# spencerkent/vision-transform-codes

Hardware: AMD Instinct MI355X
Metric: patches/sec through 200-iter FISTA + dict update, 1024-atom dict (higher is better)
Workload: dtype f16x3

## Files before the change

### vision-transform-codes_amd/csrc/fc_fused.hip

```cpp
#include "fc_fused.h"
#include "fused_common.h"

#include <stdlib.h>
#include <mutex>
#include <vector>

namespace vtc {

struct FusedParams {
  const float* images;
  const float* init;
  float* codes;
  const uint4* packA[2];
  const uint4* packT[2];
  const float* betas;
  int64_t b;
  int s;
  int num_iters;
  int fista;
  float eta, cutoff;
  const float* eta_dev;
  float lam;
  const float* dscale;
  unsigned long long* stamps;
// ... 355 lines not shown
      const float cn = Y[p][e] + Gp[e];
      Y[p][e] = cn;
      cn4[k] = cn;
      if (k == 3) {
        if (p < CREG) {
#pragma unroll
          for (int q = 0; q < 4; ++q) Cr[p < CREG ? p : 0][4 * g + q] = cn4[q];
        } else {
          *reinterpret_cast<float4*>(Cst + cst_ln + (p - CREG) * 16384 +
                                     g * 1024) =
              make_float4(cn4[0], cn4[1], cn4[2], cn4[3]);
        }
      }
      return;
    }
    if (k == 0) {
      if (p < CREG) {
        cold4 = make_float4(Cr[p < CREG ? p : 0][4 * g + 0],
                            Cr[p < CREG ? p : 0][4 * g + 1],
                            Cr[p < CREG ? p : 0][4 * g + 2],
                            Cr[p < CREG ? p : 0][4 * g + 3]);
      } else {
        cold4 = *reinterpret_cast<const float4*>(
            Cst + cst_ln + (p - CREG) * 16384 + g * 1024);
      }
    }
    const float co = (k == 0) ? cold4.x : (k == 1) ? cold4.y
                   : (k == 2) ? cold4.z : cold4.w;
    const float c = sub_rn(Y[p][e], mul_rn(eta, Gp[e]));
    const float cn = shrink_fast<MODE>(c, cutoff_l);
    Y[p][e] = fista ? add_rn(cn, mul_rn(beta, sub_rn(cn, co))) : cn;
    cn4[k] = cn;
    if (k == 3) {
      if (p < CREG) {
#pragma unroll
        for (int q = 0; q < 4; ++q) Cr[p < CREG ? p : 0][4 * g + q] = cn4[q];
      } else {
        *reinterpret_cast<float4*>(Cst + cst_ln + (p - CREG) * 16384 +
                                   g * 1024) =
            make_float4(cn4[0], cn4[1], cn4[2], cn4[3]);
      }
      const float v4[4] = {Y[p][4 * g], Y[p][4 * g + 1], Y[p][4 * g + 2],
                           Y[p][4 * g + 3]};
      uint2 hi, lo;
      split_packed<F16, 4, NP == 2>(v4, hi, lo);
      char* dst = Yx + (p & 1) * NP * kYxPart + yx_wr + 16 * g;
      *reinterpret_cast<uint2*>(dst) = hi;
      if (NP == 2) *reinterpret_cast<uint2*>(dst + kYxPart) = lo;
    }
  };

  auto step1 = [&](int p, int sg, bool overlap, float beta) {
    f32x16& G = Gb[p & 1];
#pragma unroll
    for (int e = 0; e < 16; ++e) G[e] = 0.f;
    uint4 rb_next[NP];
#pragma unroll
    for (int part = 0; part < NP; ++part)
      rb_next[part] =
          *reinterpret_cast<const uint4*>(Rx + part * kRxPart + rx_rd);
#pragma unroll
    for (int i = 0; i < 16; ++i) {
      uint4 rb[NP];
#pragma unroll
      for (int part = 0; part < NP; ++part) {
        rb[part] = rb_next[part];
        if (i + 1 < 16)
          rb_next[part] = *reinterpret_cast<const uint4*>(
              Rx + part * kRxPart + rx_rd + 32 * (i + 1));
      }
      G = mfma16<F16>(ring[0][i % RING], rb[0], G);
      if constexpr (NP == 2) {
        G = mfma16<F16>(ring[0][i % RING], rb[1], G);
        G = mfma16<F16>(ring[1][i % RING], rb[0], G);
      }
      if (overlap) {
        epilogue_elem(p - 1, i, Gb[(p - 1) & 1], beta);
        __builtin_amdgcn_sched_barrier(0);
      }
      VTC_REFILL(sg, i)
      __builtin_amdgcn_sched_barrier(0);
    }
  };

  for (int it = 0; it < P.num_iters; ++it) {
    const float beta = fista ? P.betas[it] : 0.f;
    step1(0, 0, false, beta);
    VTC_STAMP(0)
#pragma unroll
    for (int p = 0; p < NPH; ++p) {
      if (p + 1 < NPH) {
        step1(p + 1, 2 * p + 1, true, beta);
        VTC_STAMP(0)
      }
      __syncthreads();
      VTC_STAMP(2)
      if (p + 2 == NPH) {
        step3(p, p & 1, true, 2 * p + 2, [&](int i) {
          epilogue_elem(NPH - 1, i, Gb[(NPH - 1) & 1], beta);
          __builtin_amdgcn_sched_barrier(0);
        });
      } else {
        step3(p, p & 1, true, (p + 1 < NPH) ? 2 * p + 2 : 2 * NPH - 1, nothing);
      }
      VTC_STAMP(3)
    }
    exchange_r();
    VTC_STAMP(4)
  }
  if (STAMP && lane == 0) {
#pragma unroll
    for (int k = 0; k < 5; ++k) atomicAdd(P.stamps + k, acc_t[k]);
    atomicAdd(P.stamps + 7, 1ull);
  }
#undef VTC_STAMP

#pragma unroll
  for (int p = 0; p < NPH; ++p) {
#pragma unroll
    for (int g = 0; g < 4; ++g) {
      float4 v;
      if (p < CREG) {
        v = make_float4(Cr[p < CREG ? p : 0][4 * g + 0],
                        Cr[p < CREG ? p : 0][4 * g + 1],
                        Cr[p < CREG ? p : 0][4 * g + 2],
                        Cr[p < CREG ? p : 0][4 * g + 3]);
      } else {
        v = *reinterpret_cast<const float4*>(Cst + cst_ln +
                                             (p - CREG) * 16384 + g * 1024);
      }
      if (F16) {
        v.x *= inv_sigma_y;
        v.y *= inv_sigma_y;
        v.z *= inv_sigma_y;
        v.w *= inv_sigma_y;
      }
      if (live)
        *reinterpret_cast<float4*>(P.codes + patch * s + kPhaseAtoms * p +
                                   32 * w + 8 * g + 4 * h) = v;
    }
  }
#undef VTC_LOAD_A
#undef VTC_LOAD_T
#undef VTC_LOAD_SEG
#undef VTC_REFILL
#undef VTC_SEG_IS_T
#undef VTC_SEG_PHASE
}

template <int NPH, int NP, int MODE, bool F16 = false, bool STAMP = false,
          int SCHED = 0>
__global__ __launch_bounds__(256, 1) void fused_fista_kernel16(FusedParams P) {
  static_assert(!F16 || NP == 2, "the f16 split exists as three products only");
  static_assert(SCHED >= 0 && SCHED < 4, "two schedule bits");
  constexpr bool SPREAD = (SCHED & 1) != 0 && NPH > 2;
  constexpr bool EARLY_R = (SCHED & 2) != 0;
  using L = FusedLds<NPH, NP>;
  constexpr int CREG = L::CREG;
  constexpr int CR = CREG > 0 ? CREG : 1;
  constexpr int RING = (NP == 1) ? 16 : 8;
  constexpr int NPROD = (NP == 2) ? 3 : 1;
  extern __shared__ __attribute__((aligned(16))) char smem[];
  char* Cst = smem;
  char* Yx = smem + L::cst_bytes;
  char* Rx = Yx + L::yx_bytes;
  float* Stat = reinterpret_cast<float*>(Rx + L::rx_bytes);

  const int tid = threadIdx.x;
  const int lane = tid & 63;
  const int w = __builtin_amdgcn_readfirstlane(tid >> 6);
  const int c = lane & 15, q = lane >> 4;
  int64_t patch[2];
  bool live[2];
#pragma unroll
  for (int n = 0; n < 2; ++n) {
    patch[n] = (int64_t)blockIdx.x * kFP + 16 * n + c;
    live[n] = patch[n] < P.b;
  }
  const int s = P.s;

  const unsigned pack_bytes_total = (unsigned)s * kFN * 2u;
  const unsigned a_wave_off = (unsigned)w * (16u * 64u * 16u);
  const unsigned t_wave_off = (unsigned)(4 * w) * (4u * 64u * 16u);
  __amdgpu_buffer_rsrc_t rsA[NP], rsT[NP];
#pragma unroll
  for (int part = 0; part < NP; ++part) {
    rsA[part] = __builtin_amdgcn_make_buffer_rsrc(
        (void*)((const char*)P.packA[part] + a_wave_off), 0,
        (int)(pack_bytes_total - a_wave_off), 0x00020000);
    rsT[part] = __builtin_amdgcn_make_buffer_rsrc(
        (void*)((const char*)P.packT[part] + t_wave_off), 0,
        (int)(pack_bytes_total - t_wave_off), 0x00020000);
  }
  const unsigned frag_voff = (unsigned)lane * 16u;
#define VTC_LOAD_A(part, p, i) \
  buffer_load16(rsA[part], frag_voff, (unsigned)(((4 * (p)) * 16 + (i)) * 1024))
#define VTC_LOAD_T(part, p, nb, ks) \
  buffer_load16(rsT[part], frag_voff,  \
                (unsigned)((((p) * 16 + (nb)) * 4 + (ks)) * 1024))

  const int swap = ((c >> 2) ^ (c >> 3)) & 1;
  const int rd_chunk = 32 * (q >> 1) + 16 * ((q & 1) ^ swap);
  const int wr_chunk = 16 * ((q >> 1) ^ swap) + 8 * (q & 1);
  const int yx_rd = c * kYxRow + rd_chunk;
  const int yx_wr = c * kYxRow + 64 * w + wr_chunk;
  const int rx_rd = c * kRxRow + rd_chunk;
  const int rx_wr = c * kRxRow + 128 * w + wr_chunk;
  const int cst_ln = w * 4096 + lane * 16;
  constexpr int kYxHalf = 16 * kYxRow, kRxHalf = 16 * kRxRow;

  f32x16 Y[NPH];
  f32x16 Cr[CR];
  f32x4 Xr[4][2];
  f32x4 Racc[4][2];
  uint4 ring[NP][RING];

#pragma unroll
  for (int nb = 0; nb < 4; ++nb) {
#pragma unroll
    for (int n = 0; n < 2; ++n) {
      float4 v = make_float4(0.f, 0.f, 0.f, 0.f);
      if (live[n])
        v = *reinterpret_cast<const float4*>(P.images + patch[n] * kFN + 64 * w +
                                             16 * nb + 4 * q);
      Xr[nb][n][0] = v.x;
      Xr[nb][n][1] = v.y;
      Xr[nb][n][2] = v.z;
      Xr[nb][n][3] = v.w;
    }
  }
  const bool warm = (P.init != nullptr);
#pragma unroll
  for (int p = 0; p < NPH; ++p) {
#pragma unroll
    for (int g = 0; g < 4; ++g) {
      float4 v = make_float4(0.f, 0.f, 0.f, 0.f);
      if (warm && live[g & 1])
        v = *reinterpret_cast<const float4*>(P.init + patch[g & 1] * s +
                                             kPhaseAtoms * p + 32 * w +
                                             16 * (g >> 1) + 4 * q);
      Y[p][4 * g + 0] = v.x;
      Y[p][4 * g + 1] = v.y;
      Y[p][4 * g + 2] = v.z;
      Y[p][4 * g + 3] = v.w;
    }
  }
  float sigma_y[2] = {1.f, 1.f}, inv_sigma_y[2] = {1.f, 1.f};
  float sigma_d = 1.f, inv_sigma_d = 1.f;
  if (F16) {
    float sx[2] = {0.f, 0.f}, sy[2] = {0.f, 0.f};
#pragma unroll
    for (int nb = 0; nb < 4; ++nb)
#pragma unroll
      for (int n = 0; n < 2; ++n)
#pragma unroll
        for (int k = 0; k < 4; ++k) sx[n] += Xr[nb][n][k] * Xr[nb][n][k];
    if (warm) {
#pragma unroll
      for (int p = 0; p < NPH; ++p)
#pragma unroll
        for (int e = 0; e < 16; ++e) sy[(e >> 2) & 1] += Y[p][e] * Y[p][e];
    }
    float* red = reinterpret_cast<float*>(Rx);
#pragma unroll
    for (int n = 0; n < 2; ++n) {
      sx[n] += __shfl_xor(sx[n], 16, 64);
      sx[n] += __shfl_xor(sx[n], 32, 64);
      sy[n] += __shfl_xor(sy[n], 16, 64);
      sy[n] += __shfl_xor(sy[n], 32, 64);
      if (q == 0) {
        red[w * 64 + 16 * n + c] = sx[n];
        red[w * 64 + 32 + 16 * n + c] = sy[n];
      }
    }
    __syncthreads();
    float m2[2];
#pragma unroll
    for (int n = 0; n < 2; ++n) {
      float tx = 0.f, ty = 0.f;
#pragma unroll
      for (int v = 0; v < 4; ++v) {
        tx += red[v * 64 + 16 * n + c];
        ty += red[v * 64 + 32 + 16 * n + c];
      }
      m2[n] = fmaxf(tx, ty);
    }
    __syncthreads();
    sigma_d = P.dscale[0];
    inv_sigma_d = P.dscale[1];
#pragma unroll
    for (int n = 0; n < 2; ++n) {
      int e2 = 0;
      if (m2[n] > 0.f && m2[n] < __builtin_inff()) e2 = ilogbf(m2[n]) >> 1;
      e2 = e2 < -60 ? -60 : (e2 > 60 ? 60 : e2);
      sigma_y[n] = ldexpf(1.f, 8 - e2);
      inv_sigma_y[n] = ldexpf(1.f, e2 - 8);
      const float sx_scale = sigma_d * sigma_y[n];
#pragma unroll
      for (int nb = 0; nb < 4; ++nb)
#pragma unroll
        for (int k = 0; k < 4; ++k) Xr[nb][n][k] *= sx_scale;
    }
#pragma unroll
    for (int p = 0; p < NPH; ++p)
#pragma unroll
      for (int e = 0; e < 16; ++e) Y[p][e] *= sigma_y[(e >> 2) & 1];
  }
  float eta = P.eta, cutoff = P.cutoff;
  if (P.eta_dev) {
    eta = *P.eta_dev;
    cutoff = mul_rn(P.lam, eta);
  }
  float cutoff_l[2] = {cutoff, cutoff};
  if (F16) {
    eta = eta * (0.5f * inv_sigma_d);
    cutoff_l[0] = cutoff * sigma_y[0];
    cutoff_l[1] = cutoff * sigma_y[1];
  }
  const float r_scale = F16 ? 2.f * inv_sigma_d : 1.f;
  int xr_calls = 0;
#pragma unroll
  for (int p = 0; p < NPH; ++p) {
#pragma unroll
    for (int g = 0; g < 4; ++g) {
      if (p < CREG) {
#pragma unroll
        for (int k = 0; k < 4; ++k)
          Cr[p < CREG ? p : 0][4 * g + k] = Y[p][4 * g + k];
      } else {
        *reinterpret_cast<float4*>(Cst + cst_ln + (p - CREG) * 16384 +
                                   g * 1024) =
            make_float4(Y[p][4 * g + 0], Y[p][4 * g + 1], Y[p][4 * g + 2],
                        Y[p][4 * g + 3]);
      }
    }
  }
#pragma unroll
  for (int nb = 0; nb < 4; ++nb)
#pragma unroll
    for (int n = 0; n < 2; ++n)
#pragma unroll
      for (int k = 0; k < 4; ++k) Racc[nb][n][k] = 0.f;

  auto publish_group = [&](const f32x16& y, int g, int buf) {
    const float v4[4] = {y[4 * g], y[4 * g + 1], y[4 * g + 2], y[4 * g + 3]};
    uint2 hi, lo;
    split_packed<F16, 4, NP == 2>(v4, hi, lo);
    char* dst = Yx + buf * NP * kYxPart + yx_wr + 32 * (g >> 1) +
                kYxHalf * (g & 1);
    *reinterpret_cast<uint2*>(dst) = hi;
    if (NP == 2) *reinterpret_cast<uint2*>(dst + kYxPart) = lo;
  };

#define VTC_SEG_IS_T(sg) (((sg) >= 2 && ((sg) % 2) == 0) || (sg) == 2 * NPH - 1)
#define VTC_SEG_PHASE(sg)                                        \
  ((sg) == 0 ? 0                                                 \
             : (sg) == 2 * NPH - 1 ? NPH - 1                     \
                                   : ((sg) % 2 ? ((sg) + 1) / 2 : (sg) / 2 - 1))
#define VTC_SEG_BLOCK_MAJOR(sg) (EARLY_R && (sg) == 2 * NPH - 1)
#define VTC_T_NB(sg, i) \
  (VTC_SEG_BLOCK_MAJOR(sg) ? 2 * ((i) >> 3) + ((i) & 1) : (i) & 3)
#define VTC_T_KS(sg, i) (VTC_SEG_BLOCK_MAJOR(sg) ? ((i) >> 1) & 3 : (i) >> 2)
#define VTC_LOAD_SEG(part, sg, i)                                          \
  (VTC_SEG_IS_T(sg) ? VTC_LOAD_T(part, VTC_SEG_PHASE(sg), VTC_T_NB(sg, i), \
                                 VTC_T_KS(sg, i))                          \
                    : VTC_LOAD_A(part, VTC_SEG_PHASE(sg), (i)))
#define VTC_REFILL(sg, i)                                                   \
  {                                                                         \
    const int j_ = (i) + RING;                                              \
    const int sg_ = (j_ < 16) ? (sg) : (((sg) + 1) % (2 * NPH));            \
    const int i_ = (j_ < 16) ? j_ : j_ - 16;                                \
    _Pragma("unroll") for (int part = 0; part < NP; ++part)                 \
        ring[part][(i) % RING] = VTC_LOAD_SEG(part, sg_, i_);               \
  }
#define VTC_MFMA_PAIR(acc0, acc1, a, b)                                     \
  _Pragma("unroll") for (int prod = 0; prod < NPROD; ++prod) {              \
    acc0 = mfma_k32<F16>(a[prod == 2], b[0][prod == 1], acc0);              \
    acc1 = mfma_k32<F16>(a[prod == 2], b[1][prod == 1], acc1);              \
  }

  auto step3 = [&](int p, int buf, bool pipe, int sg, auto&& between) {
    uint4 yb[2][NP], yb_next[2][NP];
#pragma unroll
    for (int n = 0; n < 2; ++n)
#pragma unroll
      for (int part = 0; part < NP; ++part)
        yb_next[n][part] = *reinterpret_cast<const uint4*>(
            Yx + (buf * NP + part) * kYxPart + yx_rd + kYxHalf * n);
#pragma unroll
    for (int i = 0; i < 16; ++i) {
      const int ks = i >> 2, nb = i & 3;
      if (nb == 0) {
#pragma unroll
        for (int n = 0; n < 2; ++n)
#pragma unroll
          for (int part = 0; part < NP; ++part) yb[n][part] = yb_next[n][part];
      }
      if (nb < 2 && ks + 1 < 4) {
#pragma unroll
        for (int part = 0; part < NP; ++part)
          yb_next[nb][part] = *reinterpret_cast<const uint4*>(
              Yx + (buf * NP + part) * kYxPart + yx_rd + kYxHalf * nb +
              64 * (ks + 1));
      }
      uint4 a[NP];
#pragma unroll
      for (int part = 0; part < NP; ++part)
        a[part] = pipe ? ring[part][i % RING] : VTC_LOAD_T(part, p, nb, ks);
      VTC_MFMA_PAIR(Racc[nb][0], Racc[nb][1], a, yb)
      between(i);
      if (pipe) VTC_REFILL(sg, i)
      __builtin_amdgcn_sched_barrier(0);
    }
  };
  auto nothing = [](int) {};

  auto exchange_r = [&]() {
    float v[4][2][4];
#pragma unroll
    for (int nb = 0; nb < 4; ++nb)
#pragma unroll
      for (int n = 0; n < 2; ++n)
#pragma unroll
        for (int k = 0; k < 4; ++k) {
          v[nb][n][k] = sub_rn(Racc[nb][n][k], Xr[nb][n][k]);
          if (F16) v[nb][n][k] *= r_scale;
        }
    if (F16) {
      float f[2] = {1.f, 1.f};
#pragma unroll
      for (int n = 0; n < 2; ++n) {
        float m = 0.f;
#pragma unroll
        for (int nb = 0; nb < 4; ++nb)
#pragma unroll
          for (int k = 0; k < 4; ++k) m = fmaxf(m, fabsf(v[nb][n][k]));
        m = fmaxf(m, __shfl_xor(m, 16, 64));
        m = fmaxf(m, __shfl_xor(m, 32, 64));
        const int row = 16 * n + c;
        if (xr_calls > 0) {
          const float* prev = Stat + ((xr_calls - 1) & 1) * 128;
          const float Mx = fmaxf(fmaxf(prev[row], prev[32 + row]),
                                 fmaxf(prev[64 + row], prev[96 + row]));
          if (Mx > 2048.f && Mx < __builtin_inff())
            f[n] = ldexpf(1.f, 9 - ilogbf(Mx));
        }
        if (q == 0) Stat[(xr_calls & 1) * 128 + w * 32 + row] = m * f[n];
      }
      ++xr_calls;
      if (__any(f[0] != 1.f || f[1] != 1.f)) {
#pragma unroll
        for (int p = 0; p < NPH; ++p)
#pragma unroll
          for (int e = 0; e < 16; ++e) Y[p][e] *= f[(e >> 2) & 1];
#pragma unroll
        for (int p = 0; p < CR; ++p)
#pragma unroll
          for (int e = 0; e < 16; ++e) Cr[p][e] *= f[(e >> 2) & 1];
#pragma unroll
        for (int pl = 0; pl < L::CL; ++pl)
#pragma unroll
          for (int g = 0; g < 4; ++g) {
            float4* c4 = reinterpret_cast<float4*>(Cst + cst_ln + pl * 16384 +
                                                   g * 1024);
            float4 cc = *c4;
            const float fg = f[g & 1];
            cc.x *= fg; cc.y *= fg; cc.z *= fg; cc.w *= fg;
            *c4 = cc;
          }
#pragma unroll
        for (int n = 0; n < 2; ++n) {
#pragma unroll
          for (int nb = 0; nb < 4; ++nb)
#pragma unroll
            for (int k = 0; k < 4; ++k) {
              Xr[nb][n][k] *= f[n];
              v[nb][n][k] *= f[n];
            }
          cutoff_l[n] *= f[n];
          inv_sigma_y[n] *= 1.f / f[n];
        }
      }
    }
#pragma unroll
    for (int nb = 0; nb < 4; ++nb) {
#pragma unroll
      for (int n = 0; n < 2; ++n) {
        const float v4[4] = {v[nb][n][0], v[nb][n][1], v[nb][n][2], v[nb][n][3]};
        uint2 hi, lo;
        split_packed<F16, 4, NP == 2>(v4, hi, lo);
        char* dst = Rx + rx_wr + 32 * nb + kRxHalf * n;
        *reinterpret_cast<uint2*>(dst) = hi;
        if (NP == 2) *reinterpret_cast<uint2*>(dst + kRxPart) = lo;
      }
    }
#pragma unroll
    for (int nb = 0; nb < 4; ++nb)
#pragma unroll
      for (int n = 0; n < 2; ++n)
#pragma unroll
        for (int k = 0; k < 4; ++k) Racc[nb][n][k] = 0.f;
    __syncthreads();
  };

  float xf[2] = {1.f, 1.f}, xm[2] = {0.f, 0.f};
  auto exchange_guard = [&]() {
#pragma unroll
    for (int n = 0; n < 2; ++n) {
      xf[n] = 1.f;
      xm[n] = 0.f;
      if (F16 && xr_calls > 0) {
        const int row = 16 * n + c;
        const float* prev = Stat + ((xr_calls - 1) & 1) * 128;
        const float Mx = fmaxf(fmaxf(prev[row], prev[32 + row]),
                               fmaxf(prev[64 + row], prev[96 + row]));
        if (Mx > 2048.f && Mx < __builtin_inff())
          xf[n] = ldexpf(1.f, 9 - ilogbf(Mx));
      }
    }
  };
  float xv[4];
  auto exchange_block_a = [&](int nb, int n) {
#pragma unroll
    for (int k = 0; k < 4; ++k) {
      xv[k] = sub_rn(Racc[nb][n][k], Xr[nb][n][k]);
      if (F16) {
        xv[k] *= r_scale;
        xm[n] = fmaxf(xm[n], fabsf(xv[k]));
        xv[k] *= xf[n];
      }
      Racc[nb][n][k] = 0.f;
    }
  };
  auto exchange_block_b = [&](int nb, int n) {
    uint2 hi, lo;
    split_packed<F16, 4, NP == 2>(xv, hi, lo);
    char* dst = Rx + rx_wr + 32 * nb + kRxHalf * n;
    *reinterpret_cast<uint2*>(dst) = hi;
    if (NP == 2) *reinterpret_cast<uint2*>(dst + kRxPart) = lo;
  };
  auto exchange_block = [&](int nb, int n) {
    exchange_block_a(nb, n);
    exchange_block_b(nb, n);
  };
  auto exchange_finish = [&](int nb0) {
#pragma unroll
    for (int nb = nb0; nb < 4; ++nb)
#pragma unroll
      for (int n = 0; n < 2; ++n) exchange_block(nb, n);
    if (F16) {
#pragma unroll
      for (int n = 0; n < 2; ++n) {
        float m = xm[n];
        m = fmaxf(m, __shfl_xor(m, 16, 64));
        m = fmaxf(m, __shfl_xor(m, 32, 64));
        if (q == 0) Stat[(xr_calls & 1) * 128 + w * 32 + 16 * n + c] = m * xf[n];
      }
      ++xr_calls;
      if (__any(xf[0] != 1.f || xf[1] != 1.f)) {
#pragma unroll
        for (int p = 0; p < NPH; ++p)
#pragma unroll
          for (int e = 0; e < 16; ++e) Y[p][e] *= xf[(e >> 2) & 1];
#pragma unroll
        for (int p = 0; p < CR; ++p)
#pragma unroll
          for (int e = 0; e < 16; ++e) Cr[p][e] *= xf[(e >> 2) & 1];
#pragma unroll
        for (int pl = 0; pl < L::CL; ++pl)
#pragma unroll
          for (int g = 0; g < 4; ++g) {
            float4* c4 = reinterpret_cast<float4*>(Cst + cst_ln + pl * 16384 +
                                                   g * 1024);
            float4 cc = *c4;
            const float fg = xf[g & 1];
            cc.x *= fg; cc.y *= fg; cc.z *= fg; cc.w *= fg;
            *c4 = cc;
          }
#pragma unroll
        for (int n = 0; n < 2; ++n) {
#pragma unroll
          for (int nb = 0; nb < 4; ++nb)
#pragma unroll
            for (int k = 0; k < 4; ++k) Xr[nb][n][k] *= xf[n];
          cutoff_l[n] *= xf[n];
          inv_sigma_y[n] *= 1.f / xf[n];
        }
      }
    }
    __syncthreads();
  };

  auto step3_last = [&](int buf, int sg) {
    uint4 yb[2][NP], yb_next[2][NP];
#pragma unroll
    for (int n = 0; n < 2; ++n)
#pragma unroll
      for (int part = 0; part < NP; ++part)
        yb_next[n][part] = *reinterpret_cast<const uint4*>(
            Yx + (buf * NP + part) * kYxPart + yx_rd + kYxHalf * n);
#pragma unroll
    for (int i = 0; i < 16; ++i) {
      const int j = i & 1, nb = VTC_T_NB(sg, i);
      if (j == 0) {
#pragma unroll
        for (int n = 0; n < 2; ++n)
#pragma unroll
          for (int part = 0; part < NP; ++part) yb[n][part] = yb_next[n][part];
      }
      if (i + 2 < 16) {
#pragma unroll
        for (int part = 0; part < NP; ++part)
          yb_next[j][part] = *reinterpret_cast<const uint4*>(
              Yx + (buf * NP + part) * kYxPart + yx_rd + kYxHalf * j +
              64 * VTC_T_KS(sg, i + 2));
      }
      uint4 a[NP];
#pragma unroll
      for (int part = 0; part < NP; ++part) a[part] = ring[part][i % RING];
      VTC_MFMA_PAIR(Racc[nb][0], Racc[nb][1], a, yb)
      if (i == 6) {
        exchange_guard();
        __builtin_amdgcn_sched_barrier(0);
      }
      if (i >= 8) {
        if (j == 0)
          exchange_block_a((i - 8) >> 2, ((i - 8) >> 1) & 1);
        else
          exchange_block_b((i - 8) >> 2, ((i - 8) >> 1) & 1);
        __builtin_amdgcn_sched_barrier(0);
      }
      VTC_REFILL(sg, i)
      __builtin_amdgcn_sched_barrier(0);
    }
  };

  if (warm) {
#pragma unroll
    for (int p = 0; p < NPH; ++p) {
#pragma unroll
      for (int g = 0; g < 4; ++g) publish_group(Y[p], g, p & 1);
      __syncthreads();
      step3(p, p & 1, false, 0, nothing);
    }
  }
  exchange_r();

#pragma unroll
  for (int i = 0; i < RING; ++i)
#pragma unroll
    for (int part = 0; part < NP; ++part)
      ring[part][i] = VTC_LOAD_SEG(part, 0, i);

  const bool fista = P.fista != 0;
  unsigned long long acc_t[5] = {0, 0, 0, 0, 0};
  unsigned long long t0 = 0, t1 = 0;
#define VTC_STAMP(slot)                    \
  if (STAMP) {                             \
    t1 = stamp_now();                      \
    acc_t[slot] += t1 - t0;                \
    t0 = t1;                               \
  }
  if (STAMP) t0 = stamp_now();

  f32x4 Gb[2][4];
  float4 cold4;
  float cn4[4];

  auto epilogue_elem = [&](int p, int e, const f32x4 (&Gp)[4], float beta) {
    const int g = e >> 2, k = e & 3;
    if (MODE == 7) {
      const float cn = Y[p][e] + Gp[g][k];
      Y[p][e] = cn;
      cn4[k] = cn;
      if (k == 3) {
        if (p < CREG) {
#pragma unroll
          for (int j = 0; j < 4; ++j) Cr[p < CREG ? p : 0][4 * g + j] = cn4[j];
        } else {
          *reinterpret_cast<float4*>(Cst + cst_ln + (p - CREG) * 16384 +
                                     g * 1024) =
              make_float4(cn4[0], cn4[1], cn4[2], cn4[3]);
        }
      }
      return;
    }
    if (k == 0) {
      if (p < CREG) {
        cold4 = make_float4(Cr[p < CREG ? p : 0][4 * g + 0],
                            Cr[p < CREG ? p : 0][4 * g + 1],
                            Cr[p < CREG ? p : 0][4 * g + 2],
                            Cr[p < CREG ? p : 0][4 * g + 3]);
      } else {
        cold4 = *reinterpret_cast<const float4*>(
            Cst + cst_ln + (p - CREG) * 16384 + g * 1024);
      }
    }
    const float co = (k == 0) ? cold4.x : (k == 1) ? cold4.y
                   : (k == 2) ? cold4.z : cold4.w;
    const float cv = sub_rn(Y[p][e], mul_rn(eta, Gp[g][k]));
    const float cn = shrink_fast<MODE>(cv, cutoff_l[g & 1]);
    Y[p][e] = fista ? add_rn(cn, mul_rn(beta, sub_rn(cn, co))) : cn;
    cn4[k] = cn;
    if (k == 3) {
      if (p < CREG) {
#pragma unroll
        for (int j = 0; j < 4; ++j) Cr[p < CREG ? p : 0][4 * g + j] = cn4[j];
      } else {
        *reinterpret_cast<float4*>(Cst + cst_ln + (p - CREG) * 16384 +
                                   g * 1024) =
            make_float4(cn4[0], cn4[1], cn4[2], cn4[3]);
      }
      publish_group(Y[p], g, p & 1);
    }
  };
  auto epilogue_stage_a = [&](int p, int e, const f32x4 (&Gp)[4]) {
    const int g = e >> 2, k = e & 3;
    if (MODE == 7) {
      cn4[k] = Y[p][e] + Gp[g][k];
      return;
    }
    if (k == 0) {
      if (p < CREG) {
        cold4 = make_float4(Cr[p < CREG ? p : 0][4 * g + 0],
                            Cr[p < CREG ? p : 0][4 * g + 1],
                            Cr[p < CREG ? p : 0][4 * g + 2],
                            Cr[p < CREG ? p : 0][4 * g + 3]);
      } else {
        cold4 = *reinterpret_cast<const float4*>(
            Cst + cst_ln + (p - CREG) * 16384 + g * 1024);
      }
    }
    const float cv = sub_rn(Y[p][e], mul_rn(eta, Gp[g][k]));
    cn4[k] = shrink_fast<MODE>(cv, cutoff_l[g & 1]);
  };
  auto epilogue_stage_b = [&](int p, int e, float beta) {
    const int g = e >> 2, k = e & 3;
    const float cn = cn4[k];
    if (MODE == 7) {
      Y[p][e] = cn;
    } else {
      const float co = (k == 0) ? cold4.x : (k == 1) ? cold4.y
                     : (k == 2) ? cold4.z : cold4.w;
      Y[p][e] = fista ? add_rn(cn, mul_rn(beta, sub_rn(cn, co))) : cn;
    }
    if (k == 3) {
      if (p < CREG) {
#pragma unroll
        for (int j = 0; j < 4; ++j) Cr[p < CREG ? p : 0][4 * g + j] = cn4[j];
      } else {
        *reinterpret_cast<float4*>(Cst + cst_ln + (p - CREG) * 16384 +
                                   g * 1024) =
            make_float4(cn4[0], cn4[1], cn4[2], cn4[3]);
      }
      if (MODE != 7) publish_group(Y[p], g, p & 1);
    }
  };
  auto epilogue_half = [&](int p, int e0, int i, const f32x4 (&Gp)[4],
                           float beta) {
    if ((i & 1) == 0)
      epilogue_stage_a(p, e0 + (i >> 1), Gp);
    else
      epilogue_stage_b(p, e0 + (i >> 1), beta);
  };

  auto step1 = [&](int p, int sg, int overlap, float beta) {
    f32x4 (&G)[4] = Gb[p & 1];
#pragma unroll
    for (int g = 0; g < 4; ++g)
#pragma unroll
      for (int k = 0; k < 4; ++k) G[g][k] = 0.f;
    uint4 rb[2][NP], rb_next[2][NP];
#pragma unroll
    for (int n = 0; n < 2; ++n)
#pragma unroll
      for (int part = 0; part < NP; ++part)
        rb_next[n][part] = *reinterpret_cast<const uint4*>(
            Rx + part * kRxPart + rx_rd + kRxHalf * n);
#pragma unroll
    for (int i = 0; i < 16; ++i) {
      const int ks = i >> 1, m = i & 1;
      if (m == 0) {
#pragma unroll
        for (int n = 0; n < 2; ++n)
#pragma unroll
          for (int part = 0; part < NP; ++part) rb[n][part] = rb_next[n][part];
      }
      if (ks + 1 < 8) {
#pragma unroll
        for (int part = 0; part < NP; ++part)
          rb_next[m][part] = *reinterpret_cast<const uint4*>(
              Rx + part * kRxPart + rx_rd + kRxHalf * m + 64 * (ks + 1));
      }
      uint4 a[NP];
#pragma unroll
      for (int part = 0; part < NP; ++part) a[part] = ring[part][i % RING];
      VTC_MFMA_PAIR(G[2 * m], G[2 * m + 1], a, rb)
      if (overlap == 1) {
        epilogue_elem(p - 1, i, Gb[(p - 1) & 1], beta);
        __builtin_amdgcn_sched_barrier(0);
      } else if (overlap == 2) {
        epilogue_half(p - 1, 8, i, Gb[(p - 1) & 1], beta);
        __builtin_amdgcn_sched_barrier(0);
      }
      VTC_REFILL(sg, i)
      __builtin_amdgcn_sched_barrier(0);
    }
  };

  for (int it = 0; it < P.num_iters; ++it) {
    const float beta = fista ? P.betas[it] : 0.f;
    step1(0, 0, 0, beta);
    VTC_STAMP(0)
#pragma unroll
    for (int p = 0; p < NPH; ++p) {
      if (p + 1 < NPH) {
        step1(p + 1, 2 * p + 1, (SPREAD && p > 0) ? 2 : 1, beta);
        VTC_STAMP(0)
      }
      __syncthreads();
      VTC_STAMP(2)
      if (p + 2 == NPH) {
        step3(p, p & 1, true, 2 * p + 2, [&](int i) {
          epilogue_elem(NPH - 1, i, Gb[(NPH - 1) & 1], beta);
          __builtin_amdgcn_sched_barrier(0);
        });
      } else if (SPREAD && p + 2 < NPH) {
        step3(p, p & 1, true, 2 * p + 2, [&](int i) {
          epilogue_half(p + 1, 0, i, Gb[(p + 1) & 1], beta);
          __builtin_amdgcn_sched_barrier(0);
        });
      } else if (EARLY_R && p + 1 == NPH) {
        step3_last(p & 1, 2 * NPH - 1);
      } else {
        step3(p, p & 1, true, (p + 1 < NPH) ? 2 * p + 2 : 2 * NPH - 1, nothing);
      }
      VTC_STAMP(3)
    }
    if (EARLY_R)
      exchange_finish(2);
    else
      exchange_r();
    VTC_STAMP(4)
  }
  if (STAMP && lane == 0) {
#pragma unroll
    for (int k = 0; k < 5; ++k) atomicAdd(P.stamps + k, acc_t[k]);
    atomicAdd(P.stamps + 7, 1ull);
  }
#undef VTC_STAMP

#pragma unroll
  for (int p = 0; p < NPH; ++p) {
#pragma unroll
    for (int g = 0; g < 4; ++g) {
      float4 v;
      if (p < CREG) {
        v = make_float4(Cr[p < CREG ? p : 0][4 * g + 0],
                        Cr[p < CREG ? p : 0][4 * g + 1],
                        Cr[p < CREG ? p : 0][4 * g + 2],
                        Cr[p < CREG ? p : 0][4 * g + 3]);
      } else {
        v = *reinterpret_cast<const float4*>(Cst + cst_ln +
                                             (p - CREG) * 16384 + g * 1024);
      }
      if (F16) {
        v.x *= inv_sigma_y[g & 1];
        v.y *= inv_sigma_y[g & 1];
        v.z *= inv_sigma_y[g & 1];
        v.w *= inv_sigma_y[g & 1];
      }
      if (live[g & 1])
        *reinterpret_cast<float4*>(P.codes + patch[g & 1] * s + kPhaseAtoms * p +
                                   32 * w + 16 * (g >> 1) + 4 * q) = v;
    }
  }
#undef VTC_LOAD_A
#undef VTC_LOAD_T
#undef VTC_LOAD_SEG
#undef VTC_REFILL
#undef VTC_MFMA_PAIR
#undef VTC_SEG_IS_T
#undef VTC_SEG_PHASE
#undef VTC_SEG_BLOCK_MAJOR
#undef VTC_T_NB
#undef VTC_T_KS
}

}

namespace vtc {

static int phases_for(int64_t s) { return (int)(s / kPhaseAtoms); }

bool fused_shape_supported(int64_t b, int64_t n, int64_t s, int precision) {
  if (n != kFN || b <= 0) return false;
  if (s % kPhaseAtoms != 0) return false;
  const int nph = phases_for(s);
  if (!(nph == 2 || nph == 4 || nph == 8)) return false;
  return precision == VTC_BF16 || precision == VTC_BF16X3 ||
         precision == VTC_F16X3;
}

static int fused_parts(int precision) { return precision == VTC_BF16 ? 1 : 2; }

struct FusedLayout {
  unsigned short* packs[4] = {nullptr, nullptr, nullptr, nullptr};
  float* dscale;
  FusedLayout(Carver& ws, int64_t s, int parts) {
    for (int part = 0; part < parts; ++part) {
      packs[2 * part] = ws.take<unsigned short>((size_t)s * kFN);
      packs[2 * part + 1] = ws.take<unsigned short>((size_t)s * kFN);
    }
    dscale = ws.take<float>(2);
  }
};

size_t fused_workspace_bytes(int64_t b, int64_t n, int64_t s, int precision) {
  if (!fused_shape_supported(b, n, s, precision)) return 256;
  return measured_bytes<FusedLayout>(s, fused_parts(precision));
}

static bool default_tile16(int precision) {
  return precision == VTC_F16X3 || precision == VTC_BF16;
}
static bool use_tile16(int precision) {
  const char* v = getenv("VTC_FUSED_TILE");
  if (v && v[0] == '1' && v[1] == '6' && v[2] == 0) return true;
  if (v && v[0] == '3' && v[1] == '2' && v[2] == 0) return false;
  return default_tile16(precision);
}

template <int NP, bool F16>
constexpr int default_sched() {
  return (F16 || NP == 1) ? 1 : 0;
}
static int use_sched(int by_default) {
  const char* v = getenv("VTC_FUSED_SCHED");
  if (v && v[0] >= '0' && v[0] <= '3' && v[1] == 0) return v[0] - '0';
  return by_default;
}

template <int NPH, int NP, int MODE, bool F16, bool STAMP, bool TILE16,
          int SCHED>
static auto fused_kernel() {
  static_assert(TILE16 || SCHED == 0, "schedules exist on the 16x16x32 tile");
  if constexpr (TILE16 && SCHED != 0)
    return fused_fista_kernel16<NPH, NP, MODE, F16, STAMP, SCHED>;
  else if constexpr (TILE16)
    return fused_fista_kernel16<NPH, NP, MODE, F16, STAMP>;
  else
    return fused_fista_kernel<NPH, NP, MODE, F16, STAMP>;
}

template <int NPH, int NP, int MODE, bool F16, bool TILE16, int SCHED>
static int launch_fused(const FusedParams& P, hipStream_t st) {
  using L = FusedLds<NPH, NP>;
  auto kernel = fused_kernel<NPH, NP, MODE, F16, false, TILE16, SCHED>();
  static unsigned long long configured = 0;
  if (first_use_on_this_device(&configured)) {
    VTC_HIP_CHECK(hipFuncSetAttribute(
        reinterpret_cast<const void*>(kernel),
        hipFuncAttributeMaxDynamicSharedMemorySize, L::total));
  }
  const unsigned grid = (unsigned)ceil_div(P.b, kFP);
  hipLaunchKernelGGL(kernel, dim3(grid), dim3(256), L::total, st, P);
  VTC_LAUNCH_CHECK();
  return VTC_OK;
}

template <int NPH, int NP, bool F16, bool TILE16, int SCHED>
static int launch_stamped(FusedParams P, hipStream_t st) {
  using L = FusedLds<NPH, NP>;
  static const bool no_epilogue = getenv("VTC_FUSED_NOEPI") != nullptr;
  auto kernel =
      no_epilogue
          ? fused_kernel<NPH, NP, 7, F16, true, TILE16, SCHED>()
          : fused_kernel<NPH, NP, VTC_SOFT, F16, true, TILE16, SCHED>();
  unsigned long long* dev = nullptr;
  VTC_HIP_CHECK(hipMalloc(&dev, 8 * sizeof(unsigned long long)));
  VTC_HIP_CHECK(hipMemsetAsync(dev, 0, 8 * sizeof(unsigned long long), st));
  VTC_HIP_CHECK(hipFuncSetAttribute(
      reinterpret_cast<const void*>(kernel),
      hipFuncAttributeMaxDynamicSharedMemorySize, L::total));
  P.stamps = dev;
  hipLaunchKernelGGL(kernel, dim3((unsigned)ceil_div(P.b, kFP)), dim3(256),
                     L::total, st, P);
  VTC_LAUNCH_CHECK();
  unsigned long long host[8];
  VTC_HIP_CHECK(hipMemcpyAsync(host, dev, sizeof(host), hipMemcpyDeviceToHost,
                               st));
  VTC_HIP_CHECK(hipStreamSynchronize(st));
  VTC_HIP_CHECK(hipFree(dev));
  const char* names[5] = {"step1+epi", "epi-alone", "barrier", "step3",
                          "exchange"};
  double total = 0;
  for (int k = 0; k < 5; ++k) total += (double)host[k];
  const double per = (double)host[7] * P.num_iters * NPH;
  for (int k = 0; k < 5; ++k)
    fprintf(stderr, "[vtc stamps] %-9s %5.1f%%  %8.0f cycles/phase/wave\n",
            names[k], 100.0 * host[k] / total, host[k] / per);
  return VTC_OK;
}

template <int NPH, int NP, bool F16, bool TILE16, int SCHED>
static int dispatch_mode(const FusedParams& P, int threshold, hipStream_t st) {
  static const bool stamps = getenv("VTC_FUSED_STAMPS") != nullptr;
  if constexpr (SCHED == 0 || (NPH == 8 && NP == 2)) {
    if (stamps && threshold == VTC_SOFT && NPH == 8 && NP == 2)
      return launch_stamped<NPH, NP, F16, TILE16, SCHED>(P, st);
  }
  switch (threshold) {
    case VTC_SOFT:
      return launch_fused<NPH, NP, VTC_SOFT, F16, TILE16, SCHED>(P, st);
    case VTC_SOFT_NONNEG:
      return launch_fused<NPH, NP, VTC_SOFT_NONNEG, F16, TILE16, SCHED>(P, st);
    case VTC_HARD:
      return launch_fused<NPH, NP, VTC_HARD, F16, TILE16, SCHED>(P, st);
    default:
      return launch_fused<NPH, NP, VTC_HARD_NONNEG, F16, TILE16, SCHED>(P, st);
  }
}

template <int NPH, int NP, bool F16, bool TILE16>
static int dispatch_sched(const FusedParams& P, int threshold,
                          hipStream_t st) {
  if constexpr (TILE16) {
    const int sched = use_sched(default_sched<NP, F16>());
    if constexpr (NPH > 2) {
      if (sched == 1)
        return dispatch_mode<NPH, NP, F16, TILE16, 1>(P, threshold, st);
      if (sched == 3)
        return dispatch_mode<NPH, NP, F16, TILE16, 3>(P, threshold, st);
    }
    if (sched & 2)
      return dispatch_mode<NPH, NP, F16, TILE16, 2>(P, threshold, st);
  }
  return dispatch_mode<NPH, NP, F16, TILE16, 0>(P, threshold, st);
}

template <int NP, bool F16, bool TILE16>
static int dispatch_phases(const FusedParams& P, int threshold,
                           hipStream_t st) {
  switch (phases_for(P.s)) {
    case 2: return dispatch_sched<2, NP, F16, TILE16>(P, threshold, st);
    case 4: return dispatch_sched<4, NP, F16, TILE16>(P, threshold, st);
    case 8: return dispatch_sched<8, NP, F16, TILE16>(P, threshold, st);
  }
  set_error("fused FISTA: unsupported atom count %d", P.s);
  return VTC_ERR_UNSUPPORTED;
}

constexpr int kBetaTable = 16384;
const float* fista_beta_table_on_this_device() {
  static float* tables[64] = {nullptr};
  static std::mutex guard;
  int dev = 0;
  if (hipGetDevice(&dev) != hipSuccess || dev < 0 || dev > 63) return nullptr;
  std::lock_guard<std::mutex> lock(guard);
  if (tables[dev]) return tables[dev];
  std::vector<float> host;
  fista_betas(kBetaTable, &host);
  float* table = nullptr;
  if (hipMalloc(&table, sizeof(float) * kBetaTable) != hipSuccess)
    return nullptr;
  if (hipMemcpy(table, host.data(), sizeof(float) * kBetaTable,
                hipMemcpyHostToDevice) != hipSuccess) {
    (void)hipFree(table);
    return nullptr;
  }
  tables[dev] = table;
  return table;
}

int fused_max_iters() { return kBetaTable; }

int run_fused(const float* images, const float* dictionary,
              const float* initial_codes, float* codes, int64_t b, int64_t n,
              int64_t s, float eta, const float* eta_dev,
              float sparsity_weight, int num_iters, int variant,
              int threshold, int precision, void* workspace,
              size_t workspace_bytes, int* iters_run, hipStream_t st) {
  if (!fused_shape_supported(b, n, s, precision)) {
    set_error("fused FISTA: unsupported shape");
    return VTC_ERR_UNSUPPORTED;
  }
  if (num_iters > kBetaTable) {
    set_error("fused FISTA: at most %d iterations per call", kBetaTable);
    return VTC_ERR_UNSUPPORTED;
  }
  if (!workspace ||
      workspace_bytes < fused_workspace_bytes(b, n, s, precision)) {
    set_error("fused FISTA: workspace too small");
    return VTC_ERR_WORKSPACE;
  }
  const float* betas_dev = fista_beta_table_on_this_device();
  if (!betas_dev) {
    set_error("fused FISTA: could not place the momentum table on the device");
    return VTC_ERR_HIP;
  }
  const int parts = fused_parts(precision);
  const bool f16 = (precision == VTC_F16X3);
  Carver ws(workspace);
  FusedParams P;
  const FusedLayout L(ws, s, parts);
  unsigned short* const* packs = L.packs;
  float* dscale = L.dscale;
  if (f16) {
    hipLaunchKernelGGL(dictionary_scale_kernel, dim3(1), dim3(1024), 0, st,
                       dictionary, (int64_t)s * kFN, dscale);
    VTC_LAUNCH_CHECK();
  }
  const bool tile16 = use_tile16(precision);
  auto pack = f16 ? (tile16 ? pack_dictionary_kernel<true, true>
                            : pack_dictionary_kernel<true, false>)
                  : (tile16 ? pack_dictionary_kernel<false, true>
                            : pack_dictionary_kernel<false, false>);
  hipLaunchKernelGGL(pack, dim3(256), dim3(256), 0, st, dictionary, (int)s,
                     packs[0], packs[1], packs[2], packs[3], dscale);
  VTC_LAUNCH_CHECK();
  P.images = images;
  P.init = initial_codes;
  P.codes = codes;
  for (int part = 0; part < 2; ++part) {
    P.packA[part] = reinterpret_cast<const uint4*>(packs[2 * (part % parts)]);
    P.packT[part] =
        reinterpret_cast<const uint4*>(packs[2 * (part % parts) + 1]);
  }
  P.betas = betas_dev;
  P.b = b;
  P.s = (int)s;
  P.num_iters = num_iters;
  P.fista = (variant == VTC_FISTA) ? 1 : 0;
  P.eta = eta;
  P.eta_dev = eta_dev;
  P.lam = sparsity_weight;
  P.cutoff = sparsity_weight * eta;
  P.dscale = dscale;
  P.stamps = nullptr;
  int rc;
  if (tile16)
    rc = f16          ? dispatch_phases<2, true, true>(P, threshold, st)
         : parts == 2 ? dispatch_phases<2, false, true>(P, threshold, st)
                      : dispatch_phases<1, false, true>(P, threshold, st);
  else
    rc = f16          ? dispatch_phases<2, true, false>(P, threshold, st)
         : parts == 2 ? dispatch_phases<2, false, false>(P, threshold, st)
                      : dispatch_phases<1, false, false>(P, threshold, st);
  if (rc == VTC_OK && iters_run) *iters_run = num_iters;
  return rc;
}

}

extern "C" int vtc_init(void) {
  if (!vtc::fista_beta_table_on_this_device()) {
    vtc::set_error("vtc_init: could not place the momentum table on the device");
    return VTC_ERR_HIP;
  }
  return VTC_OK;
}
```

### vision-transform-codes_amd/csrc/split_operand.h

```cpp
#pragma once

#include "common.h"

namespace vtc {

typedef __bf16 bf16x8 __attribute__((ext_vector_type(8)));
typedef __bf16 bf16x4 __attribute__((ext_vector_type(4)));
typedef _Float16 f16x8 __attribute__((ext_vector_type(8)));
typedef _Float16 f16x4 __attribute__((ext_vector_type(4)));
typedef unsigned int u32x4 __attribute__((ext_vector_type(4)));
typedef float f32x4 __attribute__((ext_vector_type(4)));

template <bool F16> struct split_part_type { typedef __bf16 type; };
template <> struct split_part_type<true> { typedef _Float16 type; };
template <int W> struct split_words;
template <> struct split_words<4> { typedef uint2 type; typedef bf16x4 bf16; };
template <> struct split_words<8> { typedef uint4 type; typedef bf16x8 bf16; };

__device__ __forceinline__ uint2 pack_words(const unsigned (&w)[2]) {
  return make_uint2(w[0], w[1]);
}
__device__ __forceinline__ uint4 pack_words(const unsigned (&w)[4]) {
  return make_uint4(w[0], w[1], w[2], w[3]);
}

template <bool F16>
__device__ __forceinline__ f32x16 mfma16(const uint4& a, const uint4& b,
                                         const f32x16& c) {
  if (F16)
    return __builtin_amdgcn_mfma_f32_32x32x16_f16(
        __builtin_bit_cast(f16x8, a), __builtin_bit_cast(f16x8, b), c, 0, 0, 0);
  return __builtin_amdgcn_mfma_f32_32x32x16_bf16(
      __builtin_bit_cast(bf16x8, a), __builtin_bit_cast(bf16x8, b), c, 0, 0, 0);
}

template <bool F16>
__device__ __forceinline__ f32x4 mfma_k32(const uint4& a, const uint4& b,
                                          const f32x4& c) {
  if (F16)
    return __builtin_amdgcn_mfma_f32_16x16x32_f16(
        __builtin_bit_cast(f16x8, a), __builtin_bit_cast(f16x8, b), c, 0, 0, 0);
  return __builtin_amdgcn_mfma_f32_16x16x32_bf16(
      __builtin_bit_cast(bf16x8, a), __builtin_bit_cast(bf16x8, b), c, 0, 0, 0);
}

template <bool F16>
__device__ __forceinline__ void split1(float x, uint16_t& hi, uint16_t& lo) {
  typedef typename split_part_type<F16>::type part;
  const part h = (part)x;
  hi = __builtin_bit_cast(uint16_t, h);
  lo = __builtin_bit_cast(uint16_t, (part)(x - (float)h));
}
template <bool F16>
__device__ __forceinline__ unsigned short split_part(float x, int lo) {
  uint16_t h, l;
  split1<F16>(x, h, l);
  return lo ? l : h;
}

template <bool F16, int W, bool LO, bool SCALED>
__device__ __forceinline__ void split_packed_as(
    const float (&v)[W], float scale, typename split_words<W>::type& hi_out,
    typename split_words<W>::type& lo_out) {
  typedef typename split_words<W>::type words;
  if (F16) {
    typedef float pair_f32 __attribute__((ext_vector_type(2)));
    typedef _Float16 pair_f16 __attribute__((ext_vector_type(2)));
    unsigned hw[W / 2], lw[W / 2];
#pragma unroll
    for (int k = 0; k < W / 2; ++k) {
      const pair_f32 x = {SCALED ? v[2 * k] * scale : v[2 * k],
                          SCALED ? v[2 * k + 1] * scale : v[2 * k + 1]};
      const pair_f16 h = __builtin_convertvector(x, pair_f16);
      hw[k] = __builtin_bit_cast(unsigned, h);
      if (LO)
        lw[k] = __builtin_bit_cast(
            unsigned, __builtin_convertvector(
                          x - __builtin_convertvector(h, pair_f32), pair_f16));
    }
    hi_out = pack_words(hw);
    if (LO) lo_out = pack_words(lw);
  } else {
    typename split_words<W>::bf16 hi, lo;
#pragma unroll
    for (int k = 0; k < W; ++k) {
      hi[k] = (__bf16)v[k];
      if (LO) lo[k] = (__bf16)(v[k] - (float)hi[k]);
    }
    hi_out = __builtin_bit_cast(words, hi);
    if (LO) lo_out = __builtin_bit_cast(words, lo);
  }
}
template <bool F16, int W, bool LO = true>
__device__ __forceinline__ void split_packed(
    const float (&v)[W], typename split_words<W>::type& hi,
    typename split_words<W>::type& lo) {
  split_packed_as<F16, W, LO, false>(v, 1.f, hi, lo);
}
template <bool F16, int W, bool LO = true>
__device__ __forceinline__ void split_packed(
    const float (&v)[W], float scale, typename split_words<W>::type& hi,
    typename split_words<W>::type& lo) {
  split_packed_as<F16, W, LO, true>(v, scale, hi, lo);
}

__device__ __forceinline__ void split3_packed(const float (&v)[4], uint2& h_out,
                                              uint2& m_out, uint2& l_out) {
  bf16x4 h, m, l;
#pragma unroll
  for (int k = 0; k < 4; ++k) {
    h[k] = (__bf16)v[k];
    const float r1 = v[k] - (float)h[k];
    m[k] = (__bf16)r1;
    l[k] = (__bf16)(r1 - (float)m[k]);
  }
  h_out = __builtin_bit_cast(uint2, h);
  m_out = __builtin_bit_cast(uint2, m);
  l_out = __builtin_bit_cast(uint2, l);
}

}
```

Baseline: 1.784 million.

## Defer f16 residual max-stat reduction into next step and use fma_mix split

```diff
diff --git a/vision-transform-codes_amd/csrc/fc_fused.hip b/vision-transform-codes_amd/csrc/fc_fused.hip
--- a/vision-transform-codes_amd/csrc/fc_fused.hip
+++ b/vision-transform-codes_amd/csrc/fc_fused.hip
@@ -531,9 +531,10 @@
           int SCHED = 0>
 __global__ __launch_bounds__(256, 1) void fused_fista_kernel16(FusedParams P) {
   static_assert(!F16 || NP == 2, "the f16 split exists as three products only");
-  static_assert(SCHED >= 0 && SCHED < 4, "two schedule bits");
+  static_assert(SCHED >= 0 && SCHED < 8, "three schedule bits");
   constexpr bool SPREAD = (SCHED & 1) != 0 && NPH > 2;
   constexpr bool EARLY_R = (SCHED & 2) != 0;
+  constexpr bool LATE_STAT = (SCHED & 4) != 0;
   using L = FusedLds<NPH, NP>;
   constexpr int CREG = L::CREG;
   constexpr int CR = CREG > 0 ? CREG : 1;
@@ -794,6 +795,42 @@
   };
   auto nothing = [](int) {};
 
+  auto rescale_state_but_x = [&](const float (&f)[2]) {
+#pragma unroll
+    for (int p = 0; p < NPH; ++p)
+#pragma unroll
+      for (int e = 0; e < 16; ++e) Y[p][e] *= f[(e >> 2) & 1];
+#pragma unroll
+    for (int p = 0; p < CR; ++p)
+#pragma unroll
+      for (int e = 0; e < 16; ++e) Cr[p][e] *= f[(e >> 2) & 1];
+#pragma unroll
+    for (int pl = 0; pl < L::CL; ++pl)
+#pragma unroll
+      for (int g = 0; g < 4; ++g) {
+        float4* c4 = reinterpret_cast<float4*>(Cst + cst_ln + pl * 16384 +
+                                               g * 1024);
+        float4 cc = *c4;
+        const float fg = f[g & 1];
+        cc.x *= fg; cc.y *= fg; cc.z *= fg; cc.w *= fg;
+        *c4 = cc;
+      }
+#pragma unroll
+    for (int n = 0; n < 2; ++n) {
+      cutoff_l[n] *= f[n];
+      inv_sigma_y[n] *= 1.f / f[n];
+    }
+  };
+  auto rescale_state = [&](const float (&f)[2]) {
+    rescale_state_but_x(f);
+#pragma unroll
+    for (int n = 0; n < 2; ++n)
+#pragma unroll
+      for (int nb = 0; nb < 4; ++nb)
+#pragma unroll
+        for (int k = 0; k < 4; ++k) Xr[nb][n][k] *= f[n];
+  };
+
   auto exchange_r = [&]() {
     float v[4][2][4];
 #pragma unroll
@@ -828,37 +865,13 @@
       }
       ++xr_calls;
       if (__any(f[0] != 1.f || f[1] != 1.f)) {
-#pragma unroll
-        for (int p = 0; p < NPH; ++p)
-#pragma unroll
-          for (int e = 0; e < 16; ++e) Y[p][e] *= f[(e >> 2) & 1];
-#pragma unroll
-        for (int p = 0; p < CR; ++p)
-#pragma unroll
-          for (int e = 0; e < 16; ++e) Cr[p][e] *= f[(e >> 2) & 1];
-#pragma unroll
-        for (int pl = 0; pl < L::CL; ++pl)
-#pragma unroll
-          for (int g = 0; g < 4; ++g) {
-            float4* c4 = reinterpret_cast<float4*>(Cst + cst_ln + pl * 16384 +
-                                                   g * 1024);
-            float4 cc = *c4;
-            const float fg = f[g & 1];
-            cc.x *= fg; cc.y *= fg; cc.z *= fg; cc.w *= fg;
-            *c4 = cc;
-          }
-#pragma unroll
-        for (int n = 0; n < 2; ++n) {
-#pragma unroll
-          for (int nb = 0; nb < 4; ++nb)
-#pragma unroll
-            for (int k = 0; k < 4; ++k) {
-              Xr[nb][n][k] *= f[n];
-              v[nb][n][k] *= f[n];
-            }
-          cutoff_l[n] *= f[n];
-          inv_sigma_y[n] *= 1.f / f[n];
-        }
+        rescale_state(f);
+#pragma unroll
+        for (int nb = 0; nb < 4; ++nb)
+#pragma unroll
+          for (int n = 0; n < 2; ++n)
+#pragma unroll
+            for (int k = 0; k < 4; ++k) v[nb][n][k] *= f[n];
       }
     }
 #pragma unroll
@@ -908,7 +921,7 @@
         xm[n] = fmaxf(xm[n], fabsf(xv[k]));
         xv[k] *= xf[n];
       }
-      Racc[nb][n][k] = 0.f;
+      if (!LATE_STAT) Racc[nb][n][k] = 0.f;
     }
   };
   auto exchange_block_b = [&](int nb, int n) {
@@ -928,46 +941,75 @@
 #pragma unroll
       for (int n = 0; n < 2; ++n) exchange_block(nb, n);
     if (F16) {
+      if (!LATE_STAT) {
+#pragma unroll
+        for (int n = 0; n < 2; ++n) {
+          float m = xm[n];
+          m = fmaxf(m, __shfl_xor(m, 16, 64));
+          m = fmaxf(m, __shfl_xor(m, 32, 64));
+          if (q == 0)
+            Stat[(xr_calls & 1) * 128 + w * 32 + 16 * n + c] = m * xf[n];
+        }
+      }
+      ++xr_calls;
+      if (__any(xf[0] != 1.f || xf[1] != 1.f)) rescale_state(xf);
+    }
+    __syncthreads();
+  };
+
+  auto exchange_boundary = [&]() {
+    bool fire = false;
+    if (F16) {
+      ++xr_calls;
+      fire = __any(xf[0] != 1.f || xf[1] != 1.f);
+      if (fire) rescale_state_but_x(xf);
+    }
+#pragma unroll
+    for (int nb = 0; nb < 4; ++nb) {
 #pragma unroll
       for (int n = 0; n < 2; ++n) {
-        float m = xm[n];
-        m = fmaxf(m, __shfl_xor(m, 16, 64));
-        m = fmaxf(m, __shfl_xor(m, 32, 64));
-        if (q == 0) Stat[(xr_calls & 1) * 128 + w * 32 + 16 * n + c] = m * xf[n];
-      }
-      ++xr_calls;
-      if (__any(xf[0] != 1.f || xf[1] != 1.f)) {
-#pragma unroll
-        for (int p = 0; p < NPH; ++p)
-#pragma unroll
-          for (int e = 0; e < 16; ++e) Y[p][e] *= xf[(e >> 2) & 1];
-#pragma unroll
-        for (int p = 0; p < CR; ++p)
-#pragma unroll
-          for (int e = 0; e < 16; ++e) Cr[p][e] *= xf[(e >> 2) & 1];
-#pragma unroll
-        for (int pl = 0; pl < L::CL; ++pl)
-#pragma unroll
-          for (int g = 0; g < 4; ++g) {
-            float4* c4 = reinterpret_cast<float4*>(Cst + cst_ln + pl * 16384 +
-                                                   g * 1024);
-            float4 cc = *c4;
-            const float fg = xf[g & 1];
-            cc.x *= fg; cc.y *= fg; cc.z *= fg; cc.w *= fg;
-            *c4 = cc;
+        float v4[4];
+#pragma unroll
+        for (int k = 0; k < 4; ++k) {
+          v4[k] = sub_rn(Racc[nb][n][k], Xr[nb][n][k]);
+          if (F16) {
+            v4[k] *= r_scale;
+            xm[n] = fmaxf(xm[n], fabsf(v4[k]));
           }
-#pragma unroll
-        for (int n = 0; n < 2; ++n) {
-#pragma unroll
-          for (int nb = 0; nb < 4; ++nb)
-#pragma unroll
-            for (int k = 0; k < 4; ++k) Xr[nb][n][k] *= xf[n];
-          cutoff_l[n] *= xf[n];
-          inv_sigma_y[n] *= 1.f / xf[n];
         }
+        if (fire) {
+#pragma unroll
+          for (int k = 0; k < 4; ++k) {
+            v4[k] *= xf[n];
+            Xr[nb][n][k] *= xf[n];
+          }
+        }
+        uint2 hi, lo;
+        split_packed<F16, 4, NP == 2>(v4, hi, lo);
+        char* dst = Rx + rx_wr + 32 * nb + kRxHalf * n;
+        *reinterpret_cast<uint2*>(dst) = hi;
+        if (NP == 2) *reinterpret_cast<uint2*>(dst + kRxPart) = lo;
       }
     }
     __syncthreads();
+  };
+  auto exchange_late = [&](int i) {
+    if (F16 && (i == 0 || i == 2)) {
+#pragma unroll
+      for (int n = 0; n < 2; ++n)
+        xm[n] = fmaxf(xm[n], __shfl_xor(xm[n], i == 0 ? 16 : 32, 64));
+    }
+    if (F16 && i == 4) {
+#pragma unroll
+      for (int n = 0; n < 2; ++n)
+        if (q == 0)
+          Stat[((xr_calls - 1) & 1) * 128 + w * 32 + 16 * n + c] =
+              xm[n] * xf[n];
+    }
+    if (i & 1) {
+#pragma unroll
+      for (int k = 0; k < 4; ++k) Racc[i >> 2][(i >> 1) & 1][k] = 0.f;
+    }
   };
 
   auto step3_last = [&](int buf, int sg) {
@@ -1023,7 +1065,15 @@
       step3(p, p & 1, false, 0, nothing);
     }
   }
-  exchange_r();
+  if (LATE_STAT) {
+    exchange_guard();
+    if (EARLY_R)
+      exchange_finish(0);
+    else
+      exchange_boundary();
+  } else {
+    exchange_r();
+  }
 
 #pragma unroll
   for (int i = 0; i < RING; ++i)
@@ -1181,6 +1231,9 @@
       } else if (overlap == 2) {
         epilogue_half(p - 1, 8, i, Gb[(p - 1) & 1], beta);
         __builtin_amdgcn_sched_barrier(0);
+      } else if (overlap == 3) {
+        exchange_late(i);
+        __builtin_amdgcn_sched_barrier(0);
       }
       VTC_REFILL(sg, i)
       __builtin_amdgcn_sched_barrier(0);
@@ -1189,7 +1242,7 @@
 
   for (int it = 0; it < P.num_iters; ++it) {
     const float beta = fista ? P.betas[it] : 0.f;
-    step1(0, 0, 0, beta);
+    step1(0, 0, LATE_STAT ? 3 : 0, beta);
     VTC_STAMP(0)
 #pragma unroll
     for (int p = 0; p < NPH; ++p) {
@@ -1199,6 +1252,7 @@
       }
       __syncthreads();
       VTC_STAMP(2)
+      if (LATE_STAT && !EARLY_R && p + 1 == NPH) exchange_guard();
       if (p + 2 == NPH) {
         step3(p, p & 1, true, 2 * p + 2, [&](int i) {
           epilogue_elem(NPH - 1, i, Gb[(NPH - 1) & 1], beta);
@@ -1218,6 +1272,8 @@
     }
     if (EARLY_R)
       exchange_finish(2);
+    else if (LATE_STAT)
+      exchange_boundary();
     else
       exchange_r();
     VTC_STAMP(4)
@@ -1316,7 +1372,7 @@
 }
 static int use_sched(int by_default) {
   const char* v = getenv("VTC_FUSED_SCHED");
-  if (v && v[0] >= '0' && v[0] <= '3' && v[1] == 0) return v[0] - '0';
+  if (v && v[0] >= '0' && v[0] <= '7' && v[1] == 0) return v[0] - '0';
   return by_default;
 }
 
@@ -1405,15 +1461,20 @@
 static int dispatch_sched(const FusedParams& P, int threshold,
                           hipStream_t st) {
   if constexpr (TILE16) {
-    const int sched = use_sched(default_sched<NP, F16>());
+    const int sched = use_sched(default_sched<NP, F16>()) & (NPH > 2 ? 7 : 6);
     if constexpr (NPH > 2) {
-      if (sched == 1)
-        return dispatch_mode<NPH, NP, F16, TILE16, 1>(P, threshold, st);
-      if (sched == 3)
-        return dispatch_mode<NPH, NP, F16, TILE16, 3>(P, threshold, st);
-    }
-    if (sched & 2)
-      return dispatch_mode<NPH, NP, F16, TILE16, 2>(P, threshold, st);
+      switch (sched) {
+        case 1: return dispatch_mode<NPH, NP, F16, TILE16, 1>(P, threshold, st);
+        case 3: return dispatch_mode<NPH, NP, F16, TILE16, 3>(P, threshold, st);
+        case 5: return dispatch_mode<NPH, NP, F16, TILE16, 5>(P, threshold, st);
+        case 7: return dispatch_mode<NPH, NP, F16, TILE16, 7>(P, threshold, st);
+      }
+    }
+    switch (sched) {
+      case 2: return dispatch_mode<NPH, NP, F16, TILE16, 2>(P, threshold, st);
+      case 4: return dispatch_mode<NPH, NP, F16, TILE16, 4>(P, threshold, st);
+      case 6: return dispatch_mode<NPH, NP, F16, TILE16, 6>(P, threshold, st);
+    }
   }
   return dispatch_mode<NPH, NP, F16, TILE16, 0>(P, threshold, st);
 }
diff --git a/vision-transform-codes_amd/csrc/split_operand.h b/vision-transform-codes_amd/csrc/split_operand.h
--- a/vision-transform-codes_amd/csrc/split_operand.h
+++ b/vision-transform-codes_amd/csrc/split_operand.h
@@ -58,26 +58,74 @@
   return lo ? l : h;
 }
 
+template <int W, bool LO, bool SCALED>
+__device__ __forceinline__ void split_f16_cvt(const float (&v)[W], float scale,
+                                              unsigned (&hw)[W / 2],
+                                              unsigned (&lw)[W / 2]) {
+  typedef float pair_f32 __attribute__((ext_vector_type(2)));
+  typedef _Float16 pair_f16 __attribute__((ext_vector_type(2)));
+#pragma unroll
+  for (int k = 0; k < W / 2; ++k) {
+    const pair_f32 x = {SCALED ? v[2 * k] * scale : v[2 * k],
+                        SCALED ? v[2 * k + 1] * scale : v[2 * k + 1]};
+    const pair_f16 h = __builtin_convertvector(x, pair_f16);
+    hw[k] = __builtin_bit_cast(unsigned, h);
+    if (LO)
+      lw[k] = __builtin_bit_cast(
+          unsigned, __builtin_convertvector(
+                        x - __builtin_convertvector(h, pair_f32), pair_f16));
+  }
+}
+__device__ __forceinline__ void split_f16_mix_lo2(float x0, float x1, float x2,
+                                                  float x3, unsigned h0,
+                                                  unsigned h1, unsigned& l0,
+                                                  unsigned& l1) {
+  asm("v_fma_mixlo_f16 %0, %2, -1.0, %4 op_sel_hi:[1,0,0]\n\t"
+      "v_fma_mixlo_f16 %1, %3, -1.0, %6 op_sel_hi:[1,0,0]\n\t"
+      "v_fma_mixhi_f16 %0, %2, -1.0, %5 op_sel:[1,0,0] op_sel_hi:[1,0,0]\n\t"
+      "v_fma_mixhi_f16 %1, %3, -1.0, %7 op_sel:[1,0,0] op_sel_hi:[1,0,0]\n\t"
+      "s_nop 0"
+      : "=&v"(l0), "=&v"(l1)
+      : "v"(h0), "v"(h1), "v"(x0), "v"(x1), "v"(x2), "v"(x3));
+}
+template <int W, bool LO, bool SCALED>
+__device__ __forceinline__ void split_f16_mix(const float (&v)[W], float scale,
+                                              unsigned (&hw)[W / 2],
+                                              unsigned (&lw)[W / 2]) {
+  static_assert(W % 4 == 0, "two pairs per statement");
+  typedef float pair_f32 __attribute__((ext_vector_type(2)));
+  typedef _Float16 pair_f16 __attribute__((ext_vector_type(2)));
+#pragma unroll
+  for (int k = 0; k < W / 2; k += 2) {
+    float x[4];
+#pragma unroll
+    for (int j = 0; j < 4; ++j)
+      x[j] = SCALED ? v[2 * k + j] * scale : v[2 * k + j];
+    const pair_f32 xa = {x[0], x[1]}, xb = {x[2], x[3]};
+    hw[k] = __builtin_bit_cast(unsigned, __builtin_convertvector(xa, pair_f16));
+    hw[k + 1] =
+        __builtin_bit_cast(unsigned, __builtin_convertvector(xb, pair_f16));
+    if (LO)
+      split_f16_mix_lo2(x[0], x[1], x[2], x[3], hw[k], hw[k + 1], lw[k],
+                        lw[k + 1]);
+  }
+}
+#ifndef VTC_SPLIT_MIX
+#define VTC_SPLIT_MIX 1
+#endif
+
 template <bool F16, int W, bool LO, bool SCALED>
 __device__ __forceinline__ void split_packed_as(
     const float (&v)[W], float scale, typename split_words<W>::type& hi_out,
     typename split_words<W>::type& lo_out) {
   typedef typename split_words<W>::type words;
   if (F16) {
-    typedef float pair_f32 __attribute__((ext_vector_type(2)));
-    typedef _Float16 pair_f16 __attribute__((ext_vector_type(2)));
     unsigned hw[W / 2], lw[W / 2];
-#pragma unroll
-    for (int k = 0; k < W / 2; ++k) {
-      const pair_f32 x = {SCALED ? v[2 * k] * scale : v[2 * k],
-                          SCALED ? v[2 * k + 1] * scale : v[2 * k + 1]};
-      const pair_f16 h = __builtin_convertvector(x, pair_f16);
-      hw[k] = __builtin_bit_cast(unsigned, h);
-      if (LO)
-        lw[k] = __builtin_bit_cast(
-            unsigned, __builtin_convertvector(
-                          x - __builtin_convertvector(h, pair_f32), pair_f16));
-    }
+#if VTC_SPLIT_MIX
+    split_f16_mix<W, LO, SCALED>(v, scale, hw, lw);
+#else
+    split_f16_cvt<W, LO, SCALED>(v, scale, hw, lw);
+#endif
     hi_out = pack_words(hw);
     if (LO) lo_out = pack_words(lw);
   } else {
```

New measurement: 1.791 million, median of 6. Within noise of the previous version (+0.4%).
